# nixorokish/lodestar

Hardware: AMD Instinct MI355X
Metric: BLS signature sets verified/sec (1-8 GPUs) + p50 latency @128-set batch (higher is better)
Workload: dtype u32 (381-bit Fp, 12x32-bit Montgomery limbs); 1 GPU; cfg2: 1024 single-pubkey gossip sets per call, batchable requests, random-scalar batch in chunks of 16 requests; each of the 16 contexts submits 22 calls per pass (bls_gpu_verify_many, one device pass, chunks and verdicts per call); sets_per_call=1024, contexts_per_gpu=16, calls_per_pass=22, calls_in_flight_per_gpu=352, parallelism=shard-by-request x1

## Files before the change

lodestar_amd/build.py:

```python
from __future__ import annotations

import concurrent.futures as cf
import hashlib
import json
import os
import re
import subprocess
import sys
from pathlib import Path

ROOT = Path(__file__).resolve().parent.parent
PKG = ROOT / "lodestar_amd"
CSRC = PKG / "csrc"
OUT_DIR = PKG / "_native"
OBJ_DIR = ROOT / "build" / "obj"
LIB = OUT_DIR / "liblodestar_bls.so"
HIPCC = os.environ.get("HIPCC", "/opt/rocm/bin/hipcc")
ARCH = "gfx950"
FLAGS = ["-O3", "-std=c++17", "-fPIC", f"--offload-arch={ARCH}", "-I", str(ROOT / "include"), "-I", str(CSRC)]


def _headers_digest() -> str:
    h = hashlib.sha256()
    for p in sorted(list(CSRC.rglob("*.hpp")) + list((ROOT / "include").glob("*.h"))):
        h.update(p.name.encode())
        h.update(p.read_bytes())
    return h.hexdigest()


def sources() -> list[Path]:
    return [CSRC / "bls_gpu.hip"] + sorted((CSRC / "kernels").glob("*.hip"))


VARIANTS: dict[str, list[str] | dict[str, list[str]]] = {
}


def _variant_flags(variant: str | None, tu: str) -> list[str] | None:
    if not variant:
        return None
    v = VARIANTS[variant]
    return v if isinstance(v, list) else v.get(tu) or None


ADMISSION_BUDGET = 6 << 30
MIN_QUEUES = 4
SIMDS = 1024


def _resources(remarks: str) -> list[dict]:
    out, cur = [], None
    for line in remarks.splitlines():
        if "remark:" not in line:
            continue
        body = line.split("remark:", 1)[1].strip()
        if body.startswith("Function Name:"):
            cur = {"name": body.split(":", 1)[1].strip().split(" ")[0]}
            out.append(cur)
        elif cur is not None and body.startswith("ScratchSize"):
            cur["scratch"] = int(body.split(":", 1)[1].split()[0])
        elif cur is not None and body.startswith("Occupancy"):
            cur["occupancy"] = int(body.split(":", 1)[1].split()[0])
        elif cur is not None and body.startswith("VGPRs:"):
            cur["vgprs"] = int(body.split(":", 1)[1].split()[0])
        elif cur is not None and body.startswith("AGPRs:"):
            cur["agprs"] = int(body.split(":", 1)[1].split()[0])
        elif cur is not None and body.startswith("LDS Size"):
            cur["lds"] = int(body.split(":", 1)[1].split()[0])
    for k in out:
        k["device_scratch_bytes"] = k.get("scratch", 0) * 64 * k.get("occupancy", 1) * SIMDS
    return out


def _check_scratch(src: Path, kernels: list[dict]) -> None:
    cap = ADMISSION_BUDGET // MIN_QUEUES
    for k in kernels:
        if k["device_scratch_bytes"] > cap:
            raise SystemExit(f"{src.name}: kernel {k['name']} reserves {k['device_scratch_bytes'] >> 20} MiB of "
                             f"scratch per queue ({k.get('scratch')} B/lane x 64 x {k.get('occupancy')} waves/SIMD "
                             f"x {SIMDS} SIMDs) > {cap >> 20} MiB: fewer than {MIN_QUEUES} contexts would fit the "
                             "runtime's ~8 GiB (lodestar_amd/build.py ADMISSION_BUDGET)")


FIXTURE_TUS = ("k_sign", "k_probe", "k_peak", "k_selftest", "k_selftest_d28")
FIXTURE_KERNELS = ("k_coop_probe", "k_coop_run_test", "k_curve_op_chain", "k_tower_op_fin", "k_tower_op_mlq")


def _plain_name(mangled: str) -> str:
    m = re.match(r"_Z(\d+)", mangled)
    return mangled[m.end(): m.end() + int(m.group(1))] if m else mangled


def scratch_per_queue(table: list[dict]) -> tuple[int, str]:
    path = [k for k in table if k.get("tu") not in FIXTURE_TUS and _plain_name(k["name"]) not in FIXTURE_KERNELS]
    worst = max(path, key=lambda k: k["device_scratch_bytes"])
    fixtures = [k for k in table if k not in path]
    deepest = max(fixtures, key=lambda k: k["device_scratch_bytes"], default=None)
    if deepest is not None and deepest["device_scratch_bytes"] > worst["device_scratch_bytes"]:
        raise RuntimeError(
            f"fixture kernel {_plain_name(deepest['name'])} reserves {deepest['device_scratch_bytes']} B of scratch per "
            f"queue, more than the verify path's deepest ({_plain_name(worst['name'])}, "
            f"{worst['device_scratch_bytes']} B): the admission figure would under-count; shrink it or count it")
    return worst["device_scratch_bytes"], _plain_name(worst["name"])


def _compile(src: Path, hdr: str, verbose: bool, extra: list[str] | None = None) -> Path:
    flags = FLAGS + (extra or [])
    key = hashlib.sha256((hdr + " ".join(flags)).encode() + src.read_bytes()).hexdigest()[:16]
    obj = OBJ_DIR / f"{src.stem}.{key}.o"
    res = obj.with_suffix(".res.json")
    if obj.exists() and res.exists():
        return obj
    cmd = [HIPCC, *flags, "-Rpass-analysis=kernel-resource-usage", "-c", str(src), "-o", str(obj) + ".tmp"]
    if verbose:
        print("[build]", " ".join(cmd), flush=True)
    p = subprocess.run(cmd, capture_output=True, text=True)
    if p.returncode != 0:
# ... 33 lines not shown
    key = hashlib.sha256(_headers_digest().encode() + (ROOT / "tools" / "work_model.cpp").read_bytes()).hexdigest()
    stamp = OUT_DIR / ".work_stamp"
    if out.exists() and stamp.exists() and stamp.read_text() == key:
        return out
    sys.path.insert(0, str(ROOT / "tools"))
    import work_model

    work_model.build(out, verbose)
    stamp.write_text(key)
    return out


def build(jobs: int | None = None, verbose: bool = True, variant: str | None = None) -> Path:
    OUT_DIR.mkdir(parents=True, exist_ok=True)
    OBJ_DIR.mkdir(parents=True, exist_ok=True)
    build_coop_tables(verbose)
    build_work_model(verbose)
    hdr = _headers_digest()
    srcs = sources()
    lib = OUT_DIR / f"liblodestar_bls_{variant}.so" if variant else LIB
    jobs = jobs or min(len(srcs), os.cpu_count() or 4)
    kern_srcs, host_src = srcs[1:], srcs[0]
    with cf.ThreadPoolExecutor(max_workers=jobs) as ex:
        kobjs = list(ex.map(lambda s: _compile(s, hdr, verbose, _variant_flags(variant, s.stem)), kern_srcs))
    table = [dict(k, tu=o.stem.split(".")[0]) for o in kobjs for k in json.loads(o.with_suffix(".res.json").read_text())]
    per_queue, worst = scratch_per_queue(table)
    host_extra = (_variant_flags(variant, host_src.stem) or []) + [f"-DBLS_SCRATCH_PER_QUEUE={per_queue}ull",
                                                                  f'-DBLS_SCRATCH_WORST_KERNEL="{worst}"']
    objs = [_compile(host_src, hdr, verbose, host_extra)] + kobjs
    if verbose:
        for k in table:
            print(f"[build] {k['tu']}: {_plain_name(k['name'])}: {k.get('vgprs', 0)} VGPRs + {k.get('agprs', 0)} AGPRs, "
                  f"{k.get('lds', 0)} B LDS, {k.get('scratch', 0)} B/lane scratch, {k.get('occupancy')} waves/SIMD", flush=True)
    if not variant:
        (OUT_DIR / "kernel_resources.json").write_text(json.dumps(
            {"scratch_per_queue": per_queue, "scratch_worst_kernel": worst, "kernels": table}, indent=1))
    stamp = hashlib.sha256("".join(str(o) for o in objs).encode()).hexdigest()
    stamp_file = OUT_DIR / (f".lib_stamp_{variant}" if variant else ".lib_stamp")
    if lib.exists() and stamp_file.exists() and stamp_file.read_text() == stamp:
        return lib
    cmd = [HIPCC, f"--offload-arch={ARCH}", "-shared", "-fPIC", "-o", str(lib) + ".tmp", *map(str, objs), "-lz"]
    if verbose:
        print("[build]", " ".join(cmd), flush=True)
    subprocess.run(cmd, check=True)
    os.replace(str(lib) + ".tmp", lib)
    stamp_file.write_text(stamp)
    return lib


def build_hostsim(verbose: bool = True) -> Path:
    src = ROOT / "tests" / "native" / "hostsim.cpp"
    out = ROOT / "tests" / "native" / "libhostsim.so"
    hdr = _headers_digest()
    own = b"".join(p.read_bytes() for p in sorted(src.parent.glob("*.hpp")))
    key = hashlib.sha256(hdr.encode() + src.read_bytes() + own).hexdigest()[:16]
    stamp = out.with_suffix(".stamp")
    if out.exists() and stamp.exists() and stamp.read_text() == key:
        return out
    cmd = ["g++", "-O2", "-std=c++17", "-shared", "-fPIC", "-DBLS_COUNT_OPS", "-I", str(CSRC), "-I",
           str(ROOT / "include"), "-o", str(out), str(src)]
    if verbose:
        print("[build]", " ".join(cmd), flush=True)
    subprocess.run(cmd, check=True)
    stamp.write_text(key)
    return out


def build_fp2_rows_host(verbose: bool = True) -> Path:
    src = ROOT / "tests" / "native" / "fp2_rows_host.cpp"
    out = ROOT / "tests" / "native" / "libfp2_rows_host.so"
    key = hashlib.sha256(_headers_digest().encode() + src.read_bytes()).hexdigest()[:16]
    stamp = out.with_suffix(".stamp")
    if out.exists() and stamp.exists() and stamp.read_text() == key:
        return out
    cmd = ["g++", "-O2", "-std=c++17", "-shared", "-fPIC", "-I", str(CSRC), "-I", str(ROOT / "include"), "-o",
           str(out), str(src)]
    if verbose:
        print("[build]", " ".join(cmd), flush=True)
    subprocess.run(cmd, check=True)
    stamp.write_text(key)
    return out


def _build_host_program(name: str, deps: tuple[str, ...], verbose: bool, out: Path | None,
                        extra: list[str] | None) -> Path:
    native = ROOT / "tests" / "native"
    src = native / f"{name}.cpp"
    out = out or native / name
    key = hashlib.sha256((_headers_digest() + " ".join(extra or [])).encode() + src.read_bytes()
                         + b"".join((native / d).read_bytes() for d in deps)).hexdigest()[:16]
    stamp = out.with_suffix(".stamp")
    if out.exists() and stamp.exists() and stamp.read_text() == key:
        return out
    cmd = ["g++", "-O2", "-std=c++17", *(extra or []), "-I", str(CSRC), "-I", str(ROOT / "include"), "-o", str(out),
           str(src)]
    if verbose:
        print("[build]", " ".join(cmd), flush=True)
    subprocess.run(cmd, check=True)
    stamp.write_text(key)
    return out


def build_smsum_host(verbose: bool = True, out: Path | None = None, extra: list[str] | None = None) -> Path:
    return _build_host_program("smsum_host", (), verbose, out, extra)


def build_msm_host(verbose: bool = True, out: Path | None = None, extra: list[str] | None = None) -> Path:
    return _build_host_program("msm_host", (), verbose, out, extra)


def build_plan_host(verbose: bool = True, out: Path | None = None, extra: list[str] | None = None) -> Path:
    return _build_host_program("plan_host", ("plan_exports.hpp",), verbose, out, extra)


def build_deposit_host(verbose: bool = True, out: Path | None = None, extra: list[str] | None = None) -> Path:
    return _build_host_program("deposit_host", (), verbose, out, extra)


def build_comb_host(verbose: bool = True, out: Path | None = None, extra: list[str] | None = None) -> Path:
    return _build_host_program("comb_host", (), verbose, out, extra)


def build_pk_table_host(verbose: bool = True, out: Path | None = None, extra: list[str] | None = None) -> Path:
    return _build_host_program("pk_table_host", (), verbose, out, ["-pthread"] + (extra or []))


def build_committee_host(verbose: bool = True, out: Path | None = None, extra: list[str] | None = None) -> Path:
    return _build_host_program("committee_host", (), verbose, out, extra)


def build_span_host(verbose: bool = True, out: Path | None = None, extra: list[str] | None = None) -> Path:
    return _build_host_program("span_host", (), verbose, out, extra)


def build_cpu_baseline(verbose: bool = True) -> Path:
    out = ROOT / "oracle" / "cpu" / "libbls_cpu.so"
    cmd = ["make", "-s", "-C", str(ROOT / "oracle" / "cpu")]
    if verbose:
        print("[build]", " ".join(cmd), flush=True)
    subprocess.run(cmd, check=True)
    return out


def build_napi(verbose: bool = True) -> Path | None:
    hdr_dir = Path("/usr/include/node")
    if not (hdr_dir / "node_api.h").exists():
        return None
    src = ROOT / "integration" / "napi" / "lodestar_bls_napi.c"
    out = OUT_DIR / "lodestar_bls.node"
    key = hashlib.sha256(src.read_bytes() + (ROOT / "include" / "lodestar_bls.h").read_bytes()).hexdigest()[:16]
    stamp = OUT_DIR / ".napi_stamp"
    if out.exists() and stamp.exists() and stamp.read_text() == key:
        return out
    cmd = ["gcc", "-O2", "-shared", "-fPIC", "-I", str(hdr_dir), "-I", str(ROOT / "include"), str(src),
           "-L", str(OUT_DIR), "-llodestar_bls", "-Wl,-rpath,$ORIGIN", "-o", str(out)]
    if verbose:
        print("[build]", " ".join(cmd), flush=True)
    subprocess.run(cmd, check=True)
    stamp.write_text(key)
    return out


if __name__ == "__main__":
    if len(sys.argv) > 2 and sys.argv[1] == "--variant":
        build(variant=sys.argv[2])
        sys.exit(0)
# ... 13 lines not shown
```

lodestar_amd/csrc/bls/d28_rows.hpp:

```cpp
#pragma once

namespace bls {

#if defined(__HIP_DEVICE_COMPILE__)
__device__ __forceinline__ void d28_row_u1_asm(uint64_t* t, uint32_t a, const uint32_t* b) {
  asm volatile("v_mad_u64_u32 %0, vcc, %1, %2, %0"
               : "+v"(t[0])
               : "v"(a), "v"(b[0])
               : "vcc");
}
__device__ __forceinline__ void d28_row_s1_asm(uint64_t* t, uint32_t a, const uint32_t* b) {
  asm volatile("v_mad_i64_i32 %0, vcc, %1, %2, %0"
               : "+v"(t[0])
               : "v"(a), "v"(b[0])
               : "vcc");
}
__device__ __forceinline__ void d28_row_u2_asm(uint64_t* t, uint32_t a, const uint32_t* b) {
  asm volatile("v_mad_u64_u32 %0, vcc, %2, %3, %0\n\t"
               "v_mad_u64_u32 %1, vcc, %2, %4, %1"
               : "+v"(t[0]), "+v"(t[1])
               : "v"(a), "v"(b[0]), "v"(b[1])
               : "vcc");
}
__device__ __forceinline__ void d28_row_s2_asm(uint64_t* t, uint32_t a, const uint32_t* b) {
// ... 285 lines not shown
               "v_mad_i64_i32 %10, vcc, %13, %24, %10\n\t"
               "v_mad_i64_i32 %11, vcc, %13, %25, %11\n\t"
               "v_mad_i64_i32 %12, vcc, %13, %26, %12"
               : "+v"(t[0]), "+v"(t[1]), "+v"(t[2]), "+v"(t[3]), "+v"(t[4]), "+v"(t[5]), "+v"(t[6]), "+v"(t[7]), "+v"(t[8]), "+v"(t[9]), "+v"(t[10]), "+v"(t[11]), "+v"(t[12])
               : "v"(a), "v"(b[0]), "v"(b[1]), "v"(b[2]), "v"(b[3]), "v"(b[4]), "v"(b[5]), "v"(b[6]), "v"(b[7]), "v"(b[8]), "v"(b[9]), "v"(b[10]), "v"(b[11]), "v"(b[12])
               : "vcc");
}
__device__ __forceinline__ void d28_row_u14_asm(uint64_t* t, uint32_t a, const uint32_t* b) {
  asm volatile("v_mad_u64_u32 %0, vcc, %14, %15, %0\n\t"
               "v_mad_u64_u32 %1, vcc, %14, %16, %1\n\t"
               "v_mad_u64_u32 %2, vcc, %14, %17, %2\n\t"
               "v_mad_u64_u32 %3, vcc, %14, %18, %3\n\t"
               "v_mad_u64_u32 %4, vcc, %14, %19, %4\n\t"
               "v_mad_u64_u32 %5, vcc, %14, %20, %5\n\t"
               "v_mad_u64_u32 %6, vcc, %14, %21, %6\n\t"
               "v_mad_u64_u32 %7, vcc, %14, %22, %7\n\t"
               "v_mad_u64_u32 %8, vcc, %14, %23, %8\n\t"
               "v_mad_u64_u32 %9, vcc, %14, %24, %9\n\t"
               "v_mad_u64_u32 %10, vcc, %14, %25, %10\n\t"
               "v_mad_u64_u32 %11, vcc, %14, %26, %11\n\t"
               "v_mad_u64_u32 %12, vcc, %14, %27, %12\n\t"
               "v_mad_u64_u32 %13, vcc, %14, %28, %13"
               : "+v"(t[0]), "+v"(t[1]), "+v"(t[2]), "+v"(t[3]), "+v"(t[4]), "+v"(t[5]), "+v"(t[6]), "+v"(t[7]), "+v"(t[8]), "+v"(t[9]), "+v"(t[10]), "+v"(t[11]), "+v"(t[12]), "+v"(t[13])
               : "v"(a), "v"(b[0]), "v"(b[1]), "v"(b[2]), "v"(b[3]), "v"(b[4]), "v"(b[5]), "v"(b[6]), "v"(b[7]), "v"(b[8]), "v"(b[9]), "v"(b[10]), "v"(b[11]), "v"(b[12]), "v"(b[13])
               : "vcc");
}
__device__ __forceinline__ void d28_row_s14_asm(uint64_t* t, uint32_t a, const uint32_t* b) {
  asm volatile("v_mad_i64_i32 %0, vcc, %14, %15, %0\n\t"
               "v_mad_i64_i32 %1, vcc, %14, %16, %1\n\t"
               "v_mad_i64_i32 %2, vcc, %14, %17, %2\n\t"
               "v_mad_i64_i32 %3, vcc, %14, %18, %3\n\t"
               "v_mad_i64_i32 %4, vcc, %14, %19, %4\n\t"
               "v_mad_i64_i32 %5, vcc, %14, %20, %5\n\t"
               "v_mad_i64_i32 %6, vcc, %14, %21, %6\n\t"
               "v_mad_i64_i32 %7, vcc, %14, %22, %7\n\t"
               "v_mad_i64_i32 %8, vcc, %14, %23, %8\n\t"
               "v_mad_i64_i32 %9, vcc, %14, %24, %9\n\t"
               "v_mad_i64_i32 %10, vcc, %14, %25, %10\n\t"
               "v_mad_i64_i32 %11, vcc, %14, %26, %11\n\t"
               "v_mad_i64_i32 %12, vcc, %14, %27, %12\n\t"
               "v_mad_i64_i32 %13, vcc, %14, %28, %13"
               : "+v"(t[0]), "+v"(t[1]), "+v"(t[2]), "+v"(t[3]), "+v"(t[4]), "+v"(t[5]), "+v"(t[6]), "+v"(t[7]), "+v"(t[8]), "+v"(t[9]), "+v"(t[10]), "+v"(t[11]), "+v"(t[12]), "+v"(t[13])
               : "v"(a), "v"(b[0]), "v"(b[1]), "v"(b[2]), "v"(b[3]), "v"(b[4]), "v"(b[5]), "v"(b[6]), "v"(b[7]), "v"(b[8]), "v"(b[9]), "v"(b[10]), "v"(b[11]), "v"(b[12]), "v"(b[13])
               : "vcc");
}
__device__ __forceinline__ void d28_row_ux_asm(uint64_t* t, uint32_t a, const uint32_t* b) {
  asm volatile("v_mad_u64_u32 %0, vcc, %14, %15, %0\n\t"
               "v_mad_u64_u32 %1, vcc, %14, %16, %1\n\t"
               "v_mad_u64_u32 %2, vcc, %14, %17, %2\n\t"
               "v_mad_u64_u32 %3, vcc, %14, %18, %3\n\t"
               "v_mad_u64_u32 %4, vcc, %14, %19, %4\n\t"
               "v_mad_u64_u32 %5, vcc, %14, %20, %5\n\t"
               "v_mad_u64_u32 %6, vcc, %14, %21, %6\n\t"
               "v_mad_u64_u32 %7, vcc, %14, %22, %7\n\t"
               "v_mad_u64_u32 %8, vcc, %14, %23, %8\n\t"
               "v_mad_u64_u32 %9, vcc, %14, %24, %9\n\t"
               "v_mad_u64_u32 %10, vcc, %14, %25, %10\n\t"
               "v_mad_u64_u32 %11, vcc, %14, %26, %11\n\t"
               "v_mad_u64_u32 %12, vcc, %14, %27, %12\n\t"
               "v_mad_u64_u32 %13, vcc, %14, %28, 0"
               : "+v"(t[0]), "+v"(t[1]), "+v"(t[2]), "+v"(t[3]), "+v"(t[4]), "+v"(t[5]), "+v"(t[6]), "+v"(t[7]), "+v"(t[8]), "+v"(t[9]), "+v"(t[10]), "+v"(t[11]), "+v"(t[12]), "=&v"(t[13])
               : "v"(a), "v"(b[0]), "v"(b[1]), "v"(b[2]), "v"(b[3]), "v"(b[4]), "v"(b[5]), "v"(b[6]), "v"(b[7]), "v"(b[8]), "v"(b[9]), "v"(b[10]), "v"(b[11]), "v"(b[12]), "v"(b[13])
               : "vcc");
}
__device__ __forceinline__ void d28_row_uz_asm(uint64_t* t, uint32_t a, const uint32_t* b) {
  asm volatile("v_mad_u64_u32 %0, vcc, %14, %15, 0\n\t"
               "v_mad_u64_u32 %1, vcc, %14, %16, 0\n\t"
               "v_mad_u64_u32 %2, vcc, %14, %17, 0\n\t"
               "v_mad_u64_u32 %3, vcc, %14, %18, 0\n\t"
               "v_mad_u64_u32 %4, vcc, %14, %19, 0\n\t"
               "v_mad_u64_u32 %5, vcc, %14, %20, 0\n\t"
               "v_mad_u64_u32 %6, vcc, %14, %21, 0\n\t"
               "v_mad_u64_u32 %7, vcc, %14, %22, 0\n\t"
               "v_mad_u64_u32 %8, vcc, %14, %23, 0\n\t"
               "v_mad_u64_u32 %9, vcc, %14, %24, 0\n\t"
               "v_mad_u64_u32 %10, vcc, %14, %25, 0\n\t"
               "v_mad_u64_u32 %11, vcc, %14, %26, 0\n\t"
               "v_mad_u64_u32 %12, vcc, %14, %27, 0\n\t"
               "v_mad_u64_u32 %13, vcc, %14, %28, 0"
               : "=&v"(t[0]), "=&v"(t[1]), "=&v"(t[2]), "=&v"(t[3]), "=&v"(t[4]), "=&v"(t[5]), "=&v"(t[6]), "=&v"(t[7]), "=&v"(t[8]), "=&v"(t[9]), "=&v"(t[10]), "=&v"(t[11]), "=&v"(t[12]), "=&v"(t[13])
               : "v"(a), "v"(b[0]), "v"(b[1]), "v"(b[2]), "v"(b[3]), "v"(b[4]), "v"(b[5]), "v"(b[6]), "v"(b[7]), "v"(b[8]), "v"(b[9]), "v"(b[10]), "v"(b[11]), "v"(b[12]), "v"(b[13])
               : "vcc");
}
__device__ __forceinline__ void d28_row_p_asm(uint64_t* t, uint32_t m) {
  asm volatile("v_mad_u64_u32 %0, vcc, %14, %15, %0\n\t"
               "v_mad_u64_u32 %1, vcc, %14, %16, %1\n\t"
               "v_mad_u64_u32 %2, vcc, %14, %17, %2\n\t"
               "v_mad_u64_u32 %3, vcc, %14, %18, %3\n\t"
               "v_mad_u64_u32 %4, vcc, %14, %19, %4\n\t"
               "v_mad_u64_u32 %5, vcc, %14, %20, %5\n\t"
               "v_mad_u64_u32 %6, vcc, %14, %21, %6\n\t"
               "v_mad_u64_u32 %7, vcc, %14, %22, %7\n\t"
               "v_mad_u64_u32 %8, vcc, %14, %23, %8\n\t"
               "v_mad_u64_u32 %9, vcc, %14, %24, %9\n\t"
               "v_mad_u64_u32 %10, vcc, %14, %25, %10\n\t"
               "v_mad_u64_u32 %11, vcc, %14, %26, %11\n\t"
               "v_mad_u64_u32 %12, vcc, %14, %27, %12\n\t"
               "v_mad_u64_u32 %13, vcc, %14, %28, %13"
               : "+v"(t[0]), "+v"(t[1]), "+v"(t[2]), "+v"(t[3]), "+v"(t[4]), "+v"(t[5]), "+v"(t[6]), "+v"(t[7]), "+v"(t[8]), "+v"(t[9]), "+v"(t[10]), "+v"(t[11]), "+v"(t[12]), "+v"(t[13])
               : "v"(m), "s"(0xfffaaabu), "s"(0xfefffffu), "s"(0x3ffffb9u), "s"(0xfffeb15u), "s"(0x6241eabu), "s"(0xa0f6b0fu), "s"(0xf6730d2u), "s"(0xf38512bu), "s"(0x4774b84u), "s"(0x4bacd76u), "s"(0xba7b643u), "s"(0xe69a4b1u), "s"(0x1ea397fu), "s"(0x001a011u)
               : "vcc");
}
#endif

template <int N>
BLS_HD void d28_row_u(uint64_t* t, uint32_t a, const uint32_t* b) {
#if defined(__HIP_DEVICE_COMPILE__)
  if constexpr (N == 1) d28_row_u1_asm(t, a, b);
  else if constexpr (N == 2) d28_row_u2_asm(t, a, b);
  else if constexpr (N == 3) d28_row_u3_asm(t, a, b);
  else if constexpr (N == 4) d28_row_u4_asm(t, a, b);
  else if constexpr (N == 5) d28_row_u5_asm(t, a, b);
  else if constexpr (N == 6) d28_row_u6_asm(t, a, b);
  else if constexpr (N == 7) d28_row_u7_asm(t, a, b);
  else if constexpr (N == 8) d28_row_u8_asm(t, a, b);
  else if constexpr (N == 9) d28_row_u9_asm(t, a, b);
  else if constexpr (N == 10) d28_row_u10_asm(t, a, b);
  else if constexpr (N == 11) d28_row_u11_asm(t, a, b);
  else if constexpr (N == 12) d28_row_u12_asm(t, a, b);
  else if constexpr (N == 13) d28_row_u13_asm(t, a, b);
  else if constexpr (N == 14) d28_row_u14_asm(t, a, b);
#else
  for (int j = 0; j < N; ++j) t[j] += (uint64_t)a * b[j];
#endif
}
template <int N>
BLS_HD void d28_row_s(uint64_t* t, uint32_t a, const uint32_t* b) {
#if defined(__HIP_DEVICE_COMPILE__)
  if constexpr (N == 1) d28_row_s1_asm(t, a, b);
  else if constexpr (N == 2) d28_row_s2_asm(t, a, b);
  else if constexpr (N == 3) d28_row_s3_asm(t, a, b);
  else if constexpr (N == 4) d28_row_s4_asm(t, a, b);
  else if constexpr (N == 5) d28_row_s5_asm(t, a, b);
  else if constexpr (N == 6) d28_row_s6_asm(t, a, b);
  else if constexpr (N == 7) d28_row_s7_asm(t, a, b);
  else if constexpr (N == 8) d28_row_s8_asm(t, a, b);
  else if constexpr (N == 9) d28_row_s9_asm(t, a, b);
  else if constexpr (N == 10) d28_row_s10_asm(t, a, b);
  else if constexpr (N == 11) d28_row_s11_asm(t, a, b);
  else if constexpr (N == 12) d28_row_s12_asm(t, a, b);
  else if constexpr (N == 13) d28_row_s13_asm(t, a, b);
  else if constexpr (N == 14) d28_row_s14_asm(t, a, b);
#else
  for (int j = 0; j < N; ++j) t[j] = (uint64_t)((int64_t)t[j] + (int64_t)(int32_t)a * (int64_t)(int32_t)b[j]);
#endif
}
BLS_HD void d28_row_ux(uint64_t* t, uint32_t a, const uint32_t* b) {
#if defined(__HIP_DEVICE_COMPILE__)
  d28_row_ux_asm(t, a, b);
#else
  for (int j = 0; j < 13; ++j) t[j] += (uint64_t)a * b[j];
  t[13] = (uint64_t)a * b[13];
#endif
}
BLS_HD void d28_row_uz(uint64_t* t, uint32_t a, const uint32_t* b) {
#if defined(__HIP_DEVICE_COMPILE__)
  d28_row_uz_asm(t, a, b);
#else
  for (int j = 0; j < 14; ++j) t[j] = (uint64_t)a * b[j];
#endif
}
BLS_HD void d28_row_p(uint64_t* t, uint32_t m) {
#if defined(__HIP_DEVICE_COMPILE__)
  d28_row_p_asm(t, m);
#else
  const uint32_t p[14] = {0xfffaaabu, 0xfefffffu, 0x3ffffb9u, 0xfffeb15u, 0x6241eabu, 0xa0f6b0fu, 0xf6730d2u, 0xf38512bu, 0x4774b84u, 0x4bacd76u, 0xba7b643u, 0xe69a4b1u, 0x1ea397fu, 0x001a011u};
  for (int j = 0; j < 14; ++j) t[j] += (uint64_t)m * p[j];
#endif
}

}
```

lodestar_amd/csrc/bls/field.hpp:

```cpp
#pragma once

#include <stdint.h>
#include <string.h>

#if defined(__HIPCC__)
#include <hip/hip_runtime.h>
#define BLS_HD __host__ __device__ __forceinline__
#define BLS_NOINLINE static __host__ __device__ __attribute__((noinline))
#else
#define BLS_HD static inline
#define BLS_NOINLINE static __attribute__((noinline))
#endif

#if defined(BLS_COUNT_OPS) && !defined(__HIP_DEVICE_COMPILE__)
extern unsigned long long bls_fpm_counter;
#define BLS_COUNT_FPM() (++bls_fpm_counter)
#else
#define BLS_COUNT_FPM() ((void)0)
#endif

namespace bls {

struct Fp {
  uint32_t l[12];
// ... 484 lines not shown
      0x05ffffff4ba3e8d0ull, 0x06ffffff2295b5e9ull, 0x07ffffff0215b241ull, 0x08fffffee90e10e7ull, 0x09fffffecd3726b3ull,
      0x0afffffea44164a6ull, 0x0bfffffe81176f1dull, 0x0cfffffe6dd4425bull, 0x0c006802bff9cc2bull, 0x0b006802dff97fc7ull,
      0x0a006802fff97fc6ull, 0x090068031ff97fc5ull, 0x080068033ff97fc4ull, 0x070068035ff97fc3ull, 0x060068037ff97fc2ull,
      0x050068039ff97fc1ull, 0x04006803bff97fc0ull, 0x03006803dff97fbfull, 0x02006803fff97fbeull, 0x010068041ff97fbdull,
      0x000068043ff97fbcull, 0x0000000a90dd0484ull};
  return t[k];
}

BLS_HD Fp fp_redc_rows(uint64_t t[27]) {
#pragma unroll
  for (int i = 0; i < 13; ++i) {
    const uint32_t m = ((uint32_t)t[i] * BLS_NP28) & BLS_D28_MASK;
    d28_row_p(t + i, m);
    t[i + 1] += t[i] >> 28;
  }
  d28_row_p(t + 13, ((uint32_t)t[13] * BLS_NP28) & 0xFFFFFu);
  return fp_d28_tail(t);
}

BLS_HD void d28_rows_sum2(uint64_t t[27], const uint32_t x0[14], const uint32_t y0[14], const uint32_t x1[14],
                          const uint32_t y1[14]) {
  d28_row_uz(t, x0[0], y0);
  d28_row_u<14>(t, x1[0], y1);
#pragma unroll
  for (int i = 1; i < 14; ++i) {
    d28_row_ux(t + i, x0[i], y0);
    d28_row_u<14>(t + i, x1[i], y1);
  }
}

BLS_HD Fp2 fp2_mul_rows(const Fp& a0, const Fp& a1, const Fp& b0, const Fp& b1) {
  uint32_t x0[14], x1[14], y0[14], y1[14], ny1[14];
  fp_to_d28(a0, x0);
  fp_to_d28(a1, x1);
  fp_to_d28(b0, y0);
  fp_to_d28(b1, y1);
#pragma unroll
  for (int j = 0; j < 14; ++j) ny1[j] = 0u - y1[j];
  uint64_t t[27];
#pragma unroll
  for (int k = 0; k < 27; ++k) t[k] = c2w_col(k);
#pragma unroll
  for (int i = 0; i < 14; ++i) {
    d28_row_u<14>(t + i, x0[i], y0);
    d28_row_s<14>(t + i, x1[i], ny1);
  }
  const Fp c0 = fp_reduce_once(fp_redc_rows(t));
  BLS_PIN_FP(c0);
  BLS_SCHED_FENCE();
  d28_rows_sum2(t, x0, y1, x1, y0);
  return Fp2{c0, fp_reduce_once(fp_redc_rows(t))};
}

BLS_HD Fp2 fp2_sqr_rows(const Fp& a0, const Fp& a1) {
  uint32_t x0[14], x1[14], d0[14], r0[14], r1[14];
  fp_to_d28(a0, x0);
  fp_to_d28(a1, x1);
#pragma unroll
  for (int j = 0; j < 14; ++j) {
    d0[j] = x0[j] << 1;
    r0[j] = d0[j];
    r1[j] = 0u - (x1[j] << 1);
  }
  uint64_t t[27];
#pragma unroll
  for (int k = 0; k < 27; ++k) t[k] = c2w_col(k);
#define BLS_SQR_ROW(i)                              \
  r0[i] = x0[i];                                    \
  r1[i] = 0u - x1[i];                               \
  d28_row_u<14 - (i)>(t + 2 * (i), x0[i], r0 + (i)); \
  d28_row_s<14 - (i)>(t + 2 * (i), x1[i], r1 + (i));
  BLS_SQR_ROW(0) BLS_SQR_ROW(1) BLS_SQR_ROW(2) BLS_SQR_ROW(3) BLS_SQR_ROW(4) BLS_SQR_ROW(5) BLS_SQR_ROW(6)
  BLS_SQR_ROW(7) BLS_SQR_ROW(8) BLS_SQR_ROW(9) BLS_SQR_ROW(10) BLS_SQR_ROW(11) BLS_SQR_ROW(12) BLS_SQR_ROW(13)
#undef BLS_SQR_ROW
  const Fp c0 = fp_reduce_once(fp_redc_rows(t));
  BLS_PIN_FP(c0);
  BLS_SCHED_FENCE();
  d28_row_uz(t, d0[0], x1);
#pragma unroll
  for (int i = 1; i < 14; ++i) d28_row_ux(t + i, d0[i], x1);
  return Fp2{c0, fp_reduce_once(fp_redc_rows(t))};
}

#if defined(__HIP_DEVICE_COMPILE__)
__device__ __forceinline__ void bls_mac(uint64_t& lo, uint32_t& hi, uint32_t a, uint32_t b) {
  uint64_t cc;
  asm("v_mad_u64_u32 %0, %2, %3, %4, %0\n\t"
      "v_addc_co_u32 %1, %2, 0, %1, %2"
      : "+v"(lo), "+v"(hi), "=&s"(cc)
      : "v"(a), "v"(b));
}
__device__ __forceinline__ void bls_mac_s(uint64_t& lo, uint32_t& hi, uint32_t a, uint32_t b) {
  uint64_t cc;
  asm("v_mad_u64_u32 %0, %2, %3, %4, %0\n\t"
      "v_addc_co_u32 %1, %2, 0, %1, %2"
      : "+v"(lo), "+v"(hi), "=&s"(cc)
      : "v"(a), "s"(b));
}
__device__ __forceinline__ void bls_mac2(uint64_t& lo, uint32_t& hi, uint32_t a, uint32_t b, uint64_t& lo2,
                                         uint32_t& hi2, uint32_t m, uint32_t p) {
  uint64_t c1, c2;
  asm("v_mad_u64_u32 %0, %4, %6, %7, %0\n\t"
      "v_mad_u64_u32 %2, %5, %8, %9, %2\n\t"
      "v_addc_co_u32 %1, %4, 0, %1, %4\n\t"
      "v_addc_co_u32 %3, %5, 0, %3, %5"
      : "+v"(lo), "+v"(hi), "+v"(lo2), "+v"(hi2), "=&s"(c1), "=&s"(c2)
      : "v"(a), "v"(b), "v"(m), "s"(p));
}

#define BLS_MAC4(L, H, k, x, y0, y1, y2, y3, YC)                                                       \
  do {                                                                                             \
    uint64_t c0_, c1_, c2_, c3_;                                                                   \
    asm("v_mad_u64_u32 %0, %8, %12, %13, %0\n\t"                                                  \
        "v_mad_u64_u32 %2, %9, %12, %14, %2\n\t"                                                  \
        "v_mad_u64_u32 %4, %10, %12, %15, %4\n\t"                                                 \
        "v_mad_u64_u32 %6, %11, %12, %16, %6\n\t"                                                 \
        "v_addc_co_u32 %1, %8, 0, %1, %8\n\t"                                                     \
        "v_addc_co_u32 %3, %9, 0, %3, %9\n\t"                                                     \
        "v_addc_co_u32 %5, %10, 0, %5, %10\n\t"                                                   \
        "v_addc_co_u32 %7, %11, 0, %7, %11"                                                        \
        : "+v"(L[k]), "+v"(H[k]), "+v"(L[k + 1]), "+v"(H[k + 1]), "+v"(L[k + 2]), "+v"(H[k + 2]),   \
          "+v"(L[k + 3]), "+v"(H[k + 3]), "=&s"(c0_), "=&s"(c1_), "=&s"(c2_), "=&s"(c3_)            \
        : "v"(x), YC(y0), YC(y1), YC(y2), YC(y3));                                                  \
  } while (0)

__device__ __forceinline__ void bls_col_add(uint64_t& lo, uint32_t& hi, uint64_t c) {
  uint32_t l0 = (uint32_t)lo, l1 = (uint32_t)(lo >> 32);
  uint64_t cc;
  asm("v_add_co_u32 %0, %3, %0, %4\n\t"
      "v_addc_co_u32 %1, %3, %1, %5, %3\n\t"
      "v_addc_co_u32 %2, %3, 0, %2, %3"
      : "+v"(l0), "+v"(l1), "+v"(hi), "=&s"(cc)
      : "v"((uint32_t)c), "v"((uint32_t)(c >> 32)));
  lo = ((uint64_t)l1 << 32) | l0;
}

template <bool LAZY>
__device__ __forceinline__ Fp fp_mul_cols(const Fp& a, const Fp& b) {
  uint64_t L[24];
  uint32_t H[24];
#pragma unroll
  for (int k = 0; k < 24; ++k) {
    L[k] = 0;
    H[k] = 0;
  }
#pragma unroll
  for (int i = 0; i < 12; ++i) {
#pragma unroll
    for (int j = 0; j < 12; j += 4) BLS_MAC4(L, H, i + j, a.l[i], b.l[j], b.l[j + 1], b.l[j + 2], b.l[j + 3], "v");
  }
#pragma unroll
  for (int i = 0; i < 12; ++i) {
    const uint32_t m = (uint32_t)L[i] * BLS_NP0;
    BLS_MAC4(L, H, i, m, p_limb(0), p_limb(1), p_limb(2), p_limb(3), "s");
    const uint64_t c = (L[i] >> 32) | ((uint64_t)H[i] << 32);
    bls_col_add(L[i + 1], H[i + 1], c);
    BLS_MAC4(L, H, i + 4, m, p_limb(4), p_limb(5), p_limb(6), p_limb(7), "s");
    BLS_MAC4(L, H, i + 8, m, p_limb(8), p_limb(9), p_limb(10), p_limb(11), "s");
  }
  Fp u;
#pragma unroll
  for (int k = 12; k < 23; ++k) {
    u.l[k - 12] = (uint32_t)L[k];
    const uint64_t c = (L[k] >> 32) | ((uint64_t)H[k] << 32);
    bls_col_add(L[k + 1], H[k + 1], c);
  }
  u.l[11] = (uint32_t)L[23];
  return LAZY ? u : fp_reduce_once(u);
}
__device__ __forceinline__ Fp fp_sqr_cols(const Fp& a) {
  uint64_t L[24];
  uint32_t H[24];
#pragma unroll
  for (int k = 0; k < 24; ++k) {
    L[k] = 0;
    H[k] = 0;
  }
#pragma unroll
  for (int i = 0; i < 11; ++i) {
    int j = i + 1;
#pragma unroll
    for (; j + 3 < 12; j += 4) BLS_MAC4(L, H, i + j, a.l[i], a.l[j], a.l[j + 1], a.l[j + 2], a.l[j + 3], "v");
#pragma unroll
    for (; j < 12; ++j) bls_mac(L[i + j], H[i + j], a.l[i], a.l[j]);
  }
#pragma unroll
  for (int k = 1; k < 23; ++k) {
    H[k] = (H[k] << 1) | (uint32_t)(L[k] >> 63);
    L[k] <<= 1;
  }
#pragma unroll
  for (int i = 0; i < 12; ++i) bls_mac(L[2 * i], H[2 * i], a.l[i], a.l[i]);
#pragma unroll
  for (int i = 0; i < 12; ++i) {
    const uint32_t m = (uint32_t)L[i] * BLS_NP0;
    BLS_MAC4(L, H, i, m, p_limb(0), p_limb(1), p_limb(2), p_limb(3), "s");
    const uint64_t c = (L[i] >> 32) | ((uint64_t)H[i] << 32);
    bls_col_add(L[i + 1], H[i + 1], c);
    BLS_MAC4(L, H, i + 4, m, p_limb(4), p_limb(5), p_limb(6), p_limb(7), "s");
    BLS_MAC4(L, H, i + 8, m, p_limb(8), p_limb(9), p_limb(10), p_limb(11), "s");
  }
  Fp u;
#pragma unroll
  for (int k = 12; k < 23; ++k) {
    u.l[k - 12] = (uint32_t)L[k];
    const uint64_t c = (L[k] >> 32) | ((uint64_t)H[k] << 32);
    bls_col_add(L[k + 1], H[k + 1], c);
  }
  u.l[11] = (uint32_t)L[23];
  return fp_reduce_once(u);
}
#ifdef BLS_FP_INLINE
#define BLS_FP_MUL_ATTR static __device__ __forceinline__
#else
#define BLS_FP_MUL_ATTR BLS_NOINLINE
#endif
#if !defined(BLS_FP_D28)
BLS_FP_MUL_ATTR Fp fp_sqr_dev(Fp a) { return fp_sqr_cols(a); }
__device__ __forceinline__ Fp fp_mul_inl(const Fp& a, const Fp& b) { return fp_mul_cols<false>(a, b); }
__device__ __forceinline__ Fp fp_mul_lazy(const Fp& a, const Fp& b) { return fp_mul_cols<true>(a, b); }
#else
BLS_FP_MUL_ATTR Fp fp_sqr_dev(Fp a) { return fp_reduce_once(fp_sqr_d28_lazy(a)); }
__device__ __forceinline__ Fp fp_mul_inl(const Fp& a, const Fp& b) { return fp_reduce_once(fp_mul_d28_lazy(a, b)); }
__device__ __forceinline__ Fp fp_mul_lazy(const Fp& a, const Fp& b) { return fp_mul_d28_lazy(a, b); }
#endif
#define BLS_W12(x) uint32_t x##0, uint32_t x##1, uint32_t x##2, uint32_t x##3, uint32_t x##4, uint32_t x##5, \
                   uint32_t x##6, uint32_t x##7, uint32_t x##8, uint32_t x##9, uint32_t x##10, uint32_t x##11
#define BLS_FP_OF(x) Fp{{x##0, x##1, x##2, x##3, x##4, x##5, x##6, x##7, x##8, x##9, x##10, x##11}}
#define BLS_L12(v) (v).l[0], (v).l[1], (v).l[2], (v).l[3], (v).l[4], (v).l[5], (v).l[6], (v).l[7], (v).l[8], \
                   (v).l[9], (v).l[10], (v).l[11]
BLS_FP_MUL_ATTR Fp fp_mul_w(BLS_W12(a), BLS_W12(b)) { return fp_mul_inl(BLS_FP_OF(a), BLS_FP_OF(b)); }
BLS_FP_MUL_ATTR Fp fp_sqr_w(BLS_W12(a)) { return fp_sqr_dev(BLS_FP_OF(a)); }
__device__ __forceinline__ Fp fp_mul(const Fp& a, const Fp& b) { return fp_mul_w(BLS_L12(a), BLS_L12(b)); }
#if defined(BLS_FP_D28)
typedef __attribute__((address_space(3))) uint64_t* bls_fp2_slot_t;
typedef uint32_t bls_w24 __attribute__((ext_vector_type(24)));
__device__ __forceinline__ bls_w24 fp2_to_w24(const Fp2& a) {
  bls_w24 r;
#pragma unroll
  for (int k = 0; k < 12; ++k) {
    r[k] = a.c0.l[k];
    r[12 + k] = a.c1.l[k];
  }
  return r;
}
__device__ __forceinline__ Fp2 fp2_of_w24(const bls_w24& v) {
  Fp2 r;
#pragma unroll
  for (int k = 0; k < 12; ++k) {
    r.c0.l[k] = v[k];
    r.c1.l[k] = v[12 + k];
  }
  return r;
}
static __device__ __attribute__((noinline)) bls_w24 fp2_mul_w(BLS_W12(a), BLS_W12(c), bls_fp2_slot_t s) {
  Fp b0, b1;
#pragma unroll
  for (int k = 0; k < 6; ++k) {
    const uint64_t u = s[BLS_FP2_SLOT_LANES * k], v = s[BLS_FP2_SLOT_LANES * (6 + k)];
    b0.l[2 * k] = (uint32_t)u;
    b0.l[2 * k + 1] = (uint32_t)(u >> 32);
    b1.l[2 * k] = (uint32_t)v;
    b1.l[2 * k + 1] = (uint32_t)(v >> 32);
  }
  return fp2_to_w24(fp2_mul_rows(BLS_FP_OF(a), BLS_FP_OF(c), b0, b1));
}
static __device__ __attribute__((noinline)) bls_w24 fp2_sqr_w(BLS_W12(a), BLS_W12(c)) {
  return fp2_to_w24(fp2_sqr_rows(BLS_FP_OF(a), BLS_FP_OF(c)));
}
__device__ __forceinline__ Fp2 fp2_mul_prim(const Fp2& a, const Fp2& b) {
  __shared__ uint64_t slot[12 * BLS_FP2_SLOT_LANES];
  const bls_fp2_slot_t s = (bls_fp2_slot_t)&slot[threadIdx.x];
#pragma unroll
  for (int k = 0; k < 6; ++k) {
    s[BLS_FP2_SLOT_LANES * k] = ((uint64_t)b.c0.l[2 * k + 1] << 32) | b.c0.l[2 * k];
    s[BLS_FP2_SLOT_LANES * (6 + k)] = ((uint64_t)b.c1.l[2 * k + 1] << 32) | b.c1.l[2 * k];
  }
  return fp2_of_w24(fp2_mul_w(BLS_L12(a.c0), BLS_L12(a.c1), s));
}
__device__ __forceinline__ Fp2 fp2_sqr_prim(const Fp2& a) {
  return fp2_of_w24(fp2_sqr_w(BLS_L12(a.c0), BLS_L12(a.c1)));
}
#endif
#else
BLS_HD Fp fp_mul(const Fp& a, const Fp& b) {
  BLS_COUNT_FPM();
  typedef unsigned __int128 u128;
  uint64_t x[6], y[6], t[13];
  fp_w_load(a, x);
  fp_w_load(b, y);
  for (int k = 0; k < 13; ++k) t[k] = 0;
  for (int i = 0; i < 6; ++i) {
    uint64_t c = 0;
    for (int j = 0; j < 6; ++j) {
      const u128 v = (u128)x[i] * y[j] + t[i + j] + c;
      t[i + j] = (uint64_t)v;
      c = (uint64_t)(v >> 64);
    }
    t[i + 6] = c;
  }
  for (int i = 0; i < 6; ++i) {
    const uint64_t m = t[i] * BLS_NP0_64;
    uint64_t c = 0;
    for (int j = 0; j < 6; ++j) {
      const u128 v = (u128)m * BLS_P64[j] + t[i + j] + c;
      t[i + j] = (uint64_t)v;
      c = (uint64_t)(v >> 64);
    }
    for (int k = i + 6; k < 13 && c; ++k) {
      const u128 v = (u128)t[k] + c;
      t[k] = (uint64_t)v;
      c = (uint64_t)(v >> 64);
    }
  }
  fp_w_reduce(t + 6);
  return fp_w_store(t + 6);
}
BLS_HD Fp fp_mul_inl(const Fp& a, const Fp& b) { return fp_mul(a, b); }
BLS_HD Fp fp_mul_lazy(const Fp& a, const Fp& b) { return fp_mul(a, b); }
#endif

#if defined(__HIP_DEVICE_COMPILE__)
BLS_HD Fp fp_sqr(const Fp& a) { return fp_sqr_w(BLS_L12(a)); }
#else
BLS_HD Fp fp_sqr(const Fp& a) { return fp_mul(a, a); }
#endif

BLS_HD Fp fp_to_mont(const Fp& a) { return fp_mul(a, c_r2()); }

BLS_HD Fp fp_from_mont(const Fp& a) {
  Fp one = fp_zero();
  one.l[0] = 1;
  return fp_mul(a, one);
}

}
#include "lazy28.hpp"
namespace bls {

#if defined(__HIP_DEVICE_COMPILE__) && !defined(BLS_LAZY_POW)
#define BLS_LAZY_POW 1
#endif
#ifdef BLS_LAZY_POW
template <uint32_t (*E)(int), int BITS>
BLS_HD Fp fp_pow_const(const Fp& a) {
  return lz_pow_const<E, BITS>(a);
}
#else
template <uint32_t (*E)(int), int BITS>
BLS_HD Fp fp_pow_const(const Fp& a) {
  Fp tab[8];
// ... 510 lines not shown
```

Measured before the change: 4.336 million sets/s.

## Compute Fp2 mul/sqr via sum-of-products with single REDC per component

Replaces the Fp2 multiply and square primitives with a sum-of-products form. Each output component accumulates both partial products (a0*b0 + a1*(2p-b1), and so on) into one 27-word 28-bit-digit accumulator, then runs a single Montgomery reduction on it, instead of reducing per product or combining separately. New 13-wide row helpers and a 2p-b negation are added to feed it. The aim is to cut reductions and subtraction work in the Fp2 arithmetic that dominates pairing cost. The cost is larger intermediate accumulators and possible register pressure, plus correctness risk from lazy-bound assumptions.

```diff
diff --git a/lodestar_amd/build.py b/lodestar_amd/build.py
--- a/lodestar_amd/build.py
+++ b/lodestar_amd/build.py
@@ -32,7 +32,11 @@
     return [CSRC / "bls_gpu.hip"] + sorted((CSRC / "kernels").glob("*.hip"))
 
 
+_FP2_PRIM_TUS = ("k_chain", "k_mlq", "k_selftest_d28")
 VARIANTS: dict[str, list[str] | dict[str, list[str]]] = {
+    "fp2_offset": {tu: ["-DBLS_FP2_MUL_SUM=0", "-DBLS_FP2_SQR_SUM=0"] for tu in _FP2_PRIM_TUS},
+    "fp2_mul_offset": {tu: ["-DBLS_FP2_MUL_SUM=0"] for tu in _FP2_PRIM_TUS},
+    "fp2_sqr_offset": {tu: ["-DBLS_FP2_SQR_SUM=0"] for tu in _FP2_PRIM_TUS},
 }
 
 
@@ -232,6 +236,22 @@
     return out
 
 
+def build_fp2_sum_host(verbose: bool = True) -> Path:
+    src = ROOT / "tests" / "native" / "fp2_sum_host.cpp"
+    out = ROOT / "tests" / "native" / "libfp2_sum_host.so"
+    key = hashlib.sha256(_headers_digest().encode() + src.read_bytes()).hexdigest()[:16]
+    stamp = out.with_suffix(".stamp")
+    if out.exists() and stamp.exists() and stamp.read_text() == key:
+        return out
+    cmd = ["g++", "-O2", "-std=c++17", "-shared", "-fPIC", "-I", str(CSRC), "-I", str(ROOT / "include"), "-o",
+           str(out), str(src)]
+    if verbose:
+        print("[build]", " ".join(cmd), flush=True)
+    subprocess.run(cmd, check=True)
+    stamp.write_text(key)
+    return out
+
+
 def _build_host_program(name: str, deps: tuple[str, ...], verbose: bool, out: Path | None,
                         extra: list[str] | None) -> Path:
     native = ROOT / "tests" / "native"
diff --git a/lodestar_amd/csrc/bls/d28_rows.hpp b/lodestar_amd/csrc/bls/d28_rows.hpp
--- a/lodestar_amd/csrc/bls/d28_rows.hpp
+++ b/lodestar_amd/csrc/bls/d28_rows.hpp
@@ -391,6 +391,24 @@
                : "v"(a), "v"(b[0]), "v"(b[1]), "v"(b[2]), "v"(b[3]), "v"(b[4]), "v"(b[5]), "v"(b[6]), "v"(b[7]), "v"(b[8]), "v"(b[9]), "v"(b[10]), "v"(b[11]), "v"(b[12]), "v"(b[13])
                : "vcc");
 }
+__device__ __forceinline__ void d28_row_uz13_asm(uint64_t* t, uint32_t a, const uint32_t* b) {
+  asm volatile("v_mad_u64_u32 %0, vcc, %13, %14, 0\n\t"
+               "v_mad_u64_u32 %1, vcc, %13, %15, 0\n\t"
+               "v_mad_u64_u32 %2, vcc, %13, %16, 0\n\t"
+               "v_mad_u64_u32 %3, vcc, %13, %17, 0\n\t"
+               "v_mad_u64_u32 %4, vcc, %13, %18, 0\n\t"
+               "v_mad_u64_u32 %5, vcc, %13, %19, 0\n\t"
+               "v_mad_u64_u32 %6, vcc, %13, %20, 0\n\t"
+               "v_mad_u64_u32 %7, vcc, %13, %21, 0\n\t"
+               "v_mad_u64_u32 %8, vcc, %13, %22, 0\n\t"
+               "v_mad_u64_u32 %9, vcc, %13, %23, 0\n\t"
+               "v_mad_u64_u32 %10, vcc, %13, %24, 0\n\t"
+               "v_mad_u64_u32 %11, vcc, %13, %25, 0\n\t"
+               "v_mad_u64_u32 %12, vcc, %13, %26, 0"
+               : "=&v"(t[0]), "=&v"(t[1]), "=&v"(t[2]), "=&v"(t[3]), "=&v"(t[4]), "=&v"(t[5]), "=&v"(t[6]), "=&v"(t[7]), "=&v"(t[8]), "=&v"(t[9]), "=&v"(t[10]), "=&v"(t[11]), "=&v"(t[12])
+               : "v"(a), "v"(b[0]), "v"(b[1]), "v"(b[2]), "v"(b[3]), "v"(b[4]), "v"(b[5]), "v"(b[6]), "v"(b[7]), "v"(b[8]), "v"(b[9]), "v"(b[10]), "v"(b[11]), "v"(b[12])
+               : "vcc");
+}
 __device__ __forceinline__ void d28_row_p_asm(uint64_t* t, uint32_t m) {
   asm volatile("v_mad_u64_u32 %0, vcc, %14, %15, %0\n\t"
                "v_mad_u64_u32 %1, vcc, %14, %16, %1\n\t"
@@ -410,6 +428,53 @@
                : "v"(m), "s"(0xfffaaabu), "s"(0xfefffffu), "s"(0x3ffffb9u), "s"(0xfffeb15u), "s"(0x6241eabu), "s"(0xa0f6b0fu), "s"(0xf6730d2u), "s"(0xf38512bu), "s"(0x4774b84u), "s"(0x4bacd76u), "s"(0xba7b643u), "s"(0xe69a4b1u), "s"(0x1ea397fu), "s"(0x001a011u)
                : "vcc");
 }
+__device__ __forceinline__ void d28_row_p13_asm(uint64_t* t, uint32_t m) {
+  asm volatile("v_mad_u64_u32 %0, vcc, %13, %14, %0\n\t"
+               "v_mad_u64_u32 %1, vcc, %13, %15, %1\n\t"
+               "v_mad_u64_u32 %2, vcc, %13, %16, %2\n\t"
+               "v_mad_u64_u32 %3, vcc, %13, %17, %3\n\t"
+               "v_mad_u64_u32 %4, vcc, %13, %18, %4\n\t"
+               "v_mad_u64_u32 %5, vcc, %13, %19, %5\n\t"
+               "v_mad_u64_u32 %6, vcc, %13, %20, %6\n\t"
+               "v_mad_u64_u32 %7, vcc, %13, %21, %7\n\t"
+               "v_mad_u64_u32 %8, vcc, %13, %22, %8\n\t"
+               "v_mad_u64_u32 %9, vcc, %13, %23, %9\n\t"
+               "v_mad_u64_u32 %10, vcc, %13, %24, %10\n\t"
+               "v_mad_u64_u32 %11, vcc, %13, %25, %11\n\t"
+               "v_mad_u64_u32 %12, vcc, %13, %26, %12"
+               : "+v"(t[0]), "+v"(t[1]), "+v"(t[2]), "+v"(t[3]), "+v"(t[4]), "+v"(t[5]), "+v"(t[6]), "+v"(t[7]), "+v"(t[8]), "+v"(t[9]), "+v"(t[10]), "+v"(t[11]), "+v"(t[12])
+               : "v"(m), "s"(0xfefffffu), "s"(0x3ffffb9u), "s"(0xfffeb15u), "s"(0x6241eabu), "s"(0xa0f6b0fu), "s"(0xf6730d2u), "s"(0xf38512bu), "s"(0x4774b84u), "s"(0x4bacd76u), "s"(0xba7b643u), "s"(0xe69a4b1u), "s"(0x1ea397fu), "s"(0x001a011u)
+               : "vcc");
+}
+__device__ __forceinline__ void d28_neg2p_asm(uint32_t* r, const uint32_t* b) {
+  r[0] = 0xffff5556u;
+  r[1] = 0x73fdffffu;
+  r[2] = 0x62a7ffffu;
+  r[3] = 0x3d57fffdu;
+  r[4] = 0xed61ec48u;
+  r[5] = 0xce61a541u;
+  r[6] = 0xe70a257eu;
+  r[7] = 0xc8ee9709u;
+  r[8] = 0x869759aeu;
+  r[9] = 0x96374f6cu;
+  r[10] = 0x72ffcd34u;
+  r[11] = 0x340223d4u;
+  asm volatile("v_sub_co_u32 %0, vcc, %0, %12\n\t"
+               "v_subb_co_u32 %1, vcc, %1, %13, vcc\n\t"
+               "v_subb_co_u32 %2, vcc, %2, %14, vcc\n\t"
+               "v_subb_co_u32 %3, vcc, %3, %15, vcc\n\t"
+               "v_subb_co_u32 %4, vcc, %4, %16, vcc\n\t"
+               "v_subb_co_u32 %5, vcc, %5, %17, vcc\n\t"
+               "v_subb_co_u32 %6, vcc, %6, %18, vcc\n\t"
+               "v_subb_co_u32 %7, vcc, %7, %19, vcc\n\t"
+               "v_subb_co_u32 %8, vcc, %8, %20, vcc\n\t"
+               "v_subb_co_u32 %9, vcc, %9, %21, vcc\n\t"
+               "v_subb_co_u32 %10, vcc, %10, %22, vcc\n\t"
+               "v_subb_co_u32 %11, vcc, %11, %23, vcc"
+               : "+v"(r[0]), "+v"(r[1]), "+v"(r[2]), "+v"(r[3]), "+v"(r[4]), "+v"(r[5]), "+v"(r[6]), "+v"(r[7]), "+v"(r[8]), "+v"(r[9]), "+v"(r[10]), "+v"(r[11])
+               : "v"(b[0]), "v"(b[1]), "v"(b[2]), "v"(b[3]), "v"(b[4]), "v"(b[5]), "v"(b[6]), "v"(b[7]), "v"(b[8]), "v"(b[9]), "v"(b[10]), "v"(b[11])
+               : "vcc");
+}
 #endif
 
 template <int N>
@@ -469,6 +534,21 @@
   for (int j = 0; j < 14; ++j) t[j] = (uint64_t)a * b[j];
 #endif
 }
+BLS_HD void d28_row_uz13(uint64_t* t, uint32_t a, const uint32_t* b) {
+#if defined(__HIP_DEVICE_COMPILE__)
+  d28_row_uz13_asm(t, a, b);
+#else
+  for (int j = 0; j < 13; ++j) t[j] = (uint64_t)a * b[j];
+#endif
+}
+BLS_HD void d28_row_p13(uint64_t* t, uint32_t m) {
+#if defined(__HIP_DEVICE_COMPILE__)
+  d28_row_p13_asm(t, m);
+#else
+  const uint32_t p[13] = {0xfefffffu, 0x3ffffb9u, 0xfffeb15u, 0x6241eabu, 0xa0f6b0fu, 0xf6730d2u, 0xf38512bu, 0x4774b84u, 0x4bacd76u, 0xba7b643u, 0xe69a4b1u, 0x1ea397fu, 0x001a011u};
+  for (int j = 0; j < 13; ++j) t[j] += (uint64_t)m * p[j];
+#endif
+}
 BLS_HD void d28_row_p(uint64_t* t, uint32_t m) {
 #if defined(__HIP_DEVICE_COMPILE__)
   d28_row_p_asm(t, m);
@@ -477,5 +557,18 @@
   for (int j = 0; j < 14; ++j) t[j] += (uint64_t)m * p[j];
 #endif
 }
+BLS_HD void d28_neg2p(uint32_t* r, const uint32_t* b) {
+#if defined(__HIP_DEVICE_COMPILE__)
+  d28_neg2p_asm(r, b);
+#else
+  const uint32_t p2[12] = {0xffff5556u, 0x73fdffffu, 0x62a7ffffu, 0x3d57fffdu, 0xed61ec48u, 0xce61a541u, 0xe70a257eu, 0xc8ee9709u, 0x869759aeu, 0x96374f6cu, 0x72ffcd34u, 0x340223d4u};
+  uint64_t borrow = 0;
+  for (int k = 0; k < 12; ++k) {
+    const uint64_t d = (uint64_t)p2[k] - b[k] - borrow;
+    r[k] = (uint32_t)d;
+    borrow = d >> 63;
+  }
+#endif
+}
 
 }
diff --git a/lodestar_amd/csrc/bls/field.hpp b/lodestar_amd/csrc/bls/field.hpp
--- a/lodestar_amd/csrc/bls/field.hpp
+++ b/lodestar_amd/csrc/bls/field.hpp
@@ -590,6 +590,82 @@
   return Fp2{c0, fp_reduce_once(fp_redc_rows(t))};
 }
 
+BLS_HD Fp fp_neg_2p(const Fp& b) {
+  Fp r;
+  d28_neg2p(r.l, b.l);
+  return r;
+}
+
+#define BLS_D28_TOP(t, a, b) \
+  BLS_SCHED_FENCE();         \
+  (t) = (uint64_t)(a) * (b); \
+  BLS_SCHED_FENCE()
+#define BLS_D28_TOP_ADD(t, a, b) \
+  BLS_SCHED_FENCE();             \
+  (t) += (uint64_t)(a) * (b);    \
+  BLS_SCHED_FENCE()
+
+BLS_HD Fp fp_redc_rows_sum(uint64_t t[27]) {
+#pragma unroll
+  for (int i = 0; i < 13; ++i) {
+    const uint32_t m = ((uint32_t)t[i] * BLS_NP28) & BLS_D28_MASK;
+    d28_row_p13(t + i + 1, m);
+    BLS_D28_TOP_ADD(t[i], m, p28_digit(0));
+    t[i + 1] += t[i] >> 28;
+  }
+  const uint32_t m = ((uint32_t)t[13] * BLS_NP28) & 0xFFFFFu;
+  d28_row_p13(t + 14, m);
+  BLS_D28_TOP_ADD(t[13], m, p28_digit(0));
+  return fp_d28_tail(t);
+}
+
+BLS_HD void d28_rows_sum2_top(uint64_t t[27], const uint32_t x0[14], const uint32_t y0[14], const uint32_t* x1,
+                              const uint32_t* y1) {
+#pragma unroll
+  for (int i = 0; i < 14; ++i) {
+    if (i == 0) d28_row_uz13(t, x0[0], y0);
+    else d28_row_u<13>(t + i, x0[i], y0);
+    BLS_D28_TOP(t[i + 13], x0[i], y0[13]);
+    if (x1) {
+      d28_row_u<13>(t + i, x1[i], y1);
+      BLS_D28_TOP_ADD(t[i + 13], x1[i], y1[13]);
+    }
+  }
+}
+
+BLS_HD Fp2 fp2_mul_rows_sum(const Fp& a0, const Fp& a1, const Fp& b0, const Fp& b1) {
+  uint32_t x0[14], x1[14], y0[14], y1[14], ny1[14];
+  fp_to_d28(a0, x0);
+  fp_to_d28(a1, x1);
+  fp_to_d28(b0, y0);
+  fp_to_d28(b1, y1);
+  fp_to_d28(fp_neg_2p(b1), ny1);
+  uint64_t t[27];
+  d28_rows_sum2_top(t, x0, y0, x1, ny1);
+  const Fp c0 = fp_reduce_once(fp_redc_rows_sum(t));
+  BLS_PIN_FP(c0);
+  BLS_SCHED_FENCE();
+  d28_rows_sum2_top(t, x0, y1, x1, y0);
+  return Fp2{c0, fp_reduce_once(fp_redc_rows_sum(t))};
+}
+
+BLS_HD Fp2 fp2_sqr_rows_sum(const Fp& a0, const Fp& a1) {
+  uint32_t xs[14], xd[14], x0[14], d1[14];
+  fp_to_d28(fp_add_nr(a0, a1), xs);
+  fp_to_d28(fp_add_nr(a0, fp_neg_2p(a1)), xd);
+  fp_to_d28(a0, x0);
+  fp_to_d28(a1, d1);
+#pragma unroll
+  for (int j = 0; j < 14; ++j) d1[j] <<= 1;
+  uint64_t t[27];
+  d28_rows_sum2_top(t, xs, xd, nullptr, nullptr);
+  const Fp c0 = fp_reduce_once(fp_redc_rows_sum(t));
+  BLS_PIN_FP(c0);
+  BLS_SCHED_FENCE();
+  d28_rows_sum2_top(t, d1, x0, nullptr, nullptr);
+  return Fp2{c0, fp_reduce_once(fp_redc_rows_sum(t))};
+}
+
 #if defined(__HIP_DEVICE_COMPILE__)
 __device__ __forceinline__ void bls_mac(uint64_t& lo, uint32_t& hi, uint32_t a, uint32_t b) {
   uint64_t cc;
@@ -741,6 +817,12 @@
 BLS_FP_MUL_ATTR Fp fp_sqr_w(BLS_W12(a)) { return fp_sqr_dev(BLS_FP_OF(a)); }
 __device__ __forceinline__ Fp fp_mul(const Fp& a, const Fp& b) { return fp_mul_w(BLS_L12(a), BLS_L12(b)); }
 #if defined(BLS_FP_D28)
+#if !defined(BLS_FP2_MUL_SUM)
+#define BLS_FP2_MUL_SUM 1
+#endif
+#if !defined(BLS_FP2_SQR_SUM)
+#define BLS_FP2_SQR_SUM 1
+#endif
 typedef __attribute__((address_space(3))) uint64_t* bls_fp2_slot_t;
 typedef uint32_t bls_w24 __attribute__((ext_vector_type(24)));
 __device__ __forceinline__ bls_w24 fp2_to_w24(const Fp2& a) {
@@ -771,10 +853,18 @@
     b1.l[2 * k] = (uint32_t)v;
     b1.l[2 * k + 1] = (uint32_t)(v >> 32);
   }
+#if BLS_FP2_MUL_SUM
+  return fp2_to_w24(fp2_mul_rows_sum(BLS_FP_OF(a), BLS_FP_OF(c), b0, b1));
+#else
   return fp2_to_w24(fp2_mul_rows(BLS_FP_OF(a), BLS_FP_OF(c), b0, b1));
+#endif
 }
 static __device__ __attribute__((noinline)) bls_w24 fp2_sqr_w(BLS_W12(a), BLS_W12(c)) {
+#if BLS_FP2_SQR_SUM
+  return fp2_to_w24(fp2_sqr_rows_sum(BLS_FP_OF(a), BLS_FP_OF(c)));
+#else
   return fp2_to_w24(fp2_sqr_rows(BLS_FP_OF(a), BLS_FP_OF(c)));
+#endif
 }
 __device__ __forceinline__ Fp2 fp2_mul_prim(const Fp2& a, const Fp2& b) {
   __shared__ uint64_t slot[12 * BLS_FP2_SLOT_LANES];
```

Result: faster. 4.413 million sets/s, median of 4 (+1.8%).
